# HKUST-Aerial-Robotics/D2SLAM

Hardware: AMD Instinct MI355X
Metric: frames/sec SuperPoint+NetVLAD+match, 640x480 stereo (higher is better)
Workload: dtype f32

## Files before the change

d2slam_amd/api.py:

```python
import ctypes as C
import os
from dataclasses import dataclass, field
from typing import List, Optional

import numpy as np

from .weights import SP_LAYERS

_HERE = os.path.dirname(os.path.abspath(__file__))
LIB_PATH = os.path.join(_HERE, "lib", "libd2fe_hip.so")
DEV_LIB_PATH = os.path.join(_HERE, "lib", "libd2fe_hip_dev.so")
if os.environ.get("D2FE_LIB"):
    LIB_PATH = os.path.abspath(os.environ["D2FE_LIB"])

POSTPROC_B, POSTPROC_A = 0, 1
PREC_F32, PREC_F16X2, PREC_F32_WINO, PREC_F16 = 0, 1, 2, 3
ERR_TRUNCATED = -4
KEEP_ALL_CAP = 1024
PROF_STAGES = ["conv1a", "conv1b", "conv2a", "conv2b", "conv3a", "conv3b", "conv4a", "conv4b", "convPaDa",
               "convPb", "convDb", "softmax_cand", "select", "sample", "match", "netvlad", "lk"]


class D2FEError(RuntimeError):
    def __init__(self, code, msg):
# ... 191 lines not shown
    "d2fe_lk_stereo_workspace_bytes", "d2fe_lk_track_stereo_device", "d2fe_pipe_lk_result_get",
    "d2fe_track_default_params", "d2fe_lk_carry_list_bytes", "d2fe_lk_carry_list_offset", "d2fe_lk_carry_step_device", "d2fe_pipe_track_result_get",
    "d2fe_pipe_set_track_params", "d2fe_pipe_camera_default", "d2fe_pipe_create_camera", "d2fe_pipe_submit_depth", "d2fe_pipe_depth_result_get", "d2fe_depth_at_device", "d2fe_lk_carry_quad_step_device", "d2fe_lk_carry_neighbour_device", "d2fe_quad_track_enable", "d2fe_quad_track_result_get",
    "d2fe_detect_fast_by_region", "d2fe_good_features_to_track", "d2fe_pipe_default_config", "d2fe_pipe_create", "d2fe_pipe_destroy",
    "d2fe_pipe_lanes", "d2fe_pipe_stream_placement", "d2fe_pipe_classify_stream", "d2fe_pipe_submit", "d2fe_pipe_wait", "d2fe_pipe_profile_enable", "d2fe_pipe_profile_read",
    "d2fe_pipe_device_view", "d2fe_pipe_device_release", "d2fe_pipe_lane_stream", "d2fe_pipe_geometry", "d2fe_pipe_handle",
    "d2fe_quad_pipe_default_config", "d2fe_quad_pipe_create", "d2fe_quad_pipe_destroy", "d2fe_quad_pipe_submit", "d2fe_quad_pipe_wait",
    "d2fe_quad_pipe_lanes", "d2fe_quad_pipe_geometry", "d2fe_quad_undistort_device",
    "d2fe_quad_device_view", "d2fe_quad_device_release", "d2fe_quad_lane_stream", "d2fe_quad_handle",
    "d2fe_quad_exchange_default_config", "d2fe_quad_exchange_create", "d2fe_quad_exchange_destroy", "d2fe_quad_exchange_enqueue", "d2fe_quad_exchange_collect",
    "d2fe_quad_exchange_jobs", "d2fe_quad_exchange_pairs", "d2fe_quad_exchange_block_bytes", "d2fe_quad_exchange_stream", "d2fe_quad_exchange_gathered", "d2fe_quad_exchange_job_layout",
    "d2fe_exchange_default_config", "d2fe_exchange_create", "d2fe_exchange_destroy", "d2fe_exchange_enqueue", "d2fe_exchange_collect", "d2fe_exchange_pairs",
    "d2fe_exchange_block_bytes", "d2fe_exchange_stream", "d2fe_exchange_gathered",
    "d2fe_window_default_config", "d2fe_window_create", "d2fe_window_create_quad", "d2fe_window_destroy", "d2fe_window_stream", "d2fe_window_push",
    "d2fe_window_push_host", "d2fe_window_retain", "d2fe_window_retain_plan", "d2fe_window_size", "d2fe_window_tags", "d2fe_window_track_device", "d2fe_window_collect",
    "d2fe_loop_default_config", "d2fe_loop_create", "d2fe_loop_create_quad", "d2fe_loop_destroy", "d2fe_loop_enqueue", "d2fe_loop_collect", "d2fe_loop_ntotal",
    "d2fe_loop_keyframes", "d2fe_loop_stream", "d2fe_loop_query_device", "d2fe_loop_add_host", "d2fe_rccl_load", "d2fe_rccl_path", "d2fe_rccl_unique_id", "d2fe_rccl_comm_init_rank", "d2fe_rccl_comm_destroy"]
DEBUG_EXPORTS = [
    "d2fe_debug_graph_count", "d2fe_debug_read", "d2fe_debug_netvlad_layer", "d2fe_debug_netvlad_stamps", "d2fe_debug_pack_wino",
    "d2fe_debug_pack_netvlad", "d2fe_debug_netvlad_tile", "d2fe_debug_conv3x3_wino", "d2fe_debug_match_stamps",
    "d2fe_debug_netvlad_plan", "d2fe_debug_regime_counts", "d2fe_debug_regime_reset",
    "d2fe_debug_softmax_cand", "d2fe_debug_select_b", "d2fe_debug_sample_b", "d2fe_debug_sample_b_pca", "d2fe_debug_nms2_a"]
REGIMES = ["wino_nt1_one", "wino_nt1_static", "wino_nt1_claimed", "wino_nt2_one", "wino_nt2_static", "wino_nt2_claimed_ring", "wino_nt2_claimed_fused1b",
           "match_nw4", "match_nw2", "nv_gmerge", "nv_front_tpw", "wino_last_grid", "wino_last_total"]


def _preload_hip_runtime():
    import importlib.util
    import sys
    if "torch" in sys.modules:
        return
    try:
        spec = importlib.util.find_spec("torch")
    except (ImportError, ValueError):
        spec = None
    if spec is not None and spec.origin:
        cand = os.path.join(os.path.dirname(spec.origin), "lib", "libamdhip64.so")
        if os.path.exists(cand):
            try:
                C.CDLL(cand, mode=C.RTLD_GLOBAL)
            except OSError:
                pass


def load_library(dev=False):
    global _lib, _dev_lib
    if dev:
# ... 1694 lines not shown
```

d2slam_amd/csrc/context.h:

```cpp
#pragma once
#include <hip/hip_runtime.h>

#include <atomic>

#include <array>
#include <deque>
#include <map>
#include <memory>
#include <mutex>
#include <string>
#include <vector>

#include "../../include/d2fe.h"
#include "kernels.h"
#include "sp_plan.h"

namespace d2fe {
int ctx_fail(int code, const std::string& msg);
}

#define HIP_TRY(expr)                                                                                       \
  do {                                                                                                      \
    hipError_t e_ = (expr);                                                                                 \
    if (e_ != hipSuccess)                                                                                   \
// ... 78 lines not shown
inline bool nv_is_tail(NvKind k) { return k == NvKind::Tail || k == NvKind::TailBlock; }

struct NvLayer {
  int kind, cin, cout, cout_pad, stride, act, res; int oh = 0, ow = 0;
  int gmax = 1;
  bool materialised = false;
  float* w = nullptr; float* b = nullptr;
};
struct NvStep {
  NvKind kind = NvKind::Pw; int l0 = 0, l1 = 0;
  int halves = 1;
  bool one_slab_out = false;
  float* w0 = nullptr; float* we = nullptr; float* wp = nullptr; float* bp = nullptr;
  float* wp2 = nullptr; float* bp2 = nullptr;
};
struct NvKnobs {
  static int positive(int v, int dflt) { return v > 0 ? v : dflt; }
  bool legacy = d2fe_dev_env("D2FE_NV_LEGACY", 0) != 0;
  bool pair = d2fe_dev_env("D2FE_NV_PAIR", 1) != 0, xblock = d2fe_dev_env("D2FE_NV_XBLOCK", 1) != 0;
  int blocks_target = positive(d2fe_dev_env("D2FE_NV_BLOCKS", 0), 512);
  int tail_blocks = positive(d2fe_dev_env("D2FE_NV_TAIL_BLOCKS", 0), 30);
  int slabsum = d2fe_dev_env("D2FE_NV_SLABSUM", 3);
  bool group_rule = d2fe_dev_env("D2FE_NV_GROUP_RULE", 1) != 0;
  bool merge = d2fe_dev_env("D2FE_NV_MERGE", 1) != 0;
  int front_tpw = d2fe_dev_env("D2FE_NV_FRONT_TPW", 0), nbuf = d2fe_dev_env("D2FE_NV_NBUF", 0);
  int stamp_step = d2fe_dev_env("D2FE_NV_STAMP_STEP", -1);
};
struct NvNet {
  std::vector<NvLayer> layers;
  std::vector<NvStep> plan;
  int feat = 0, proj = 0, k = 0, feat_gmax = 1;
  float *pre_w = nullptr, *pre_b = nullptr, *aw = nullptr, *aw_pack = nullptr, *ab = nullptr, *cen = nullptr;
  float *pca_comp = nullptr, *pca_mean = nullptr; int pca_m = 0;
  NvKnobs knobs;
  NvNet() = default; NvNet(const NvNet&) = delete; NvNet& operator=(const NvNet&) = delete; ~NvNet();
};
struct NvSlabs { int n = 1; long stride = 0; };
struct NvLast { std::vector<NvSlabs> layer; NvSlabs feat; int stamp_wgs = 0; };
struct NvRun {
  std::vector<float*> out;
  float *feat_buf = nullptr, *raw = nullptr, *part = nullptr;
  unsigned long long* stamps = nullptr;
  NvLast last;
  int alloc(const NvNet& net, int max_batch);
  void release();
  NvRun() = default; NvRun(const NvRun&) = delete; NvRun& operator=(const NvRun&) = delete; ~NvRun() { release(); }
// ... 125 lines not shown
```

d2slam_amd/csrc/kernels.h:

```cpp
#pragma once
#include <hip/hip_runtime.h>
#include <stdint.h>

#ifdef D2FE_DEVTOOLS
#include <cstdlib>
static inline int d2fe_dev_env(const char* name, int dflt) { const char* e = getenv(name); return e ? atoi(e) : dflt; }
#define D2FE_ABL(a, bits) ((a).ablate & (bits))
#define D2FE_STAMP(buf, wg, i) do { if ((buf) && threadIdx.x == 0) (buf)[(size_t)(wg) * 16 + (i)] = wall_clock64(); } while (0)
#else
static inline int d2fe_dev_env(const char*, int dflt) { return dflt; }
#define D2FE_ABL(a, bits) (0)
#define D2FE_STAMP(buf, wg, i) do {} while (0)
#endif

#ifdef D2FE_DEVTOOLS
#include "../../include/d2fe_debug.h"
namespace d2fe { void regime_note(int regime); void regime_set(int regime, long long value); }
#define D2FE_REGIME(r) ::d2fe::regime_note(r)
#define D2FE_REGIME_SET(r, v) ::d2fe::regime_set(r, v)
#else
#define D2FE_REGIME(r) do {} while (0)
#define D2FE_REGIME_SET(r, v) do {} while (0)
#endif

// ... 92 lines not shown

struct NvBlockArgs {
  const float* in;
  int in_slabs; long in_slab_stride;
  const uint8_t* img; int img_stride; long img_istride; int H0, W0;
  int c0_stride, c0_pt, c0_pl, act0; const float* w0;
  float* out; long out_slab_stride;
  const float* res; int res_slabs; long res_slab_stride;
  int H, W, Cin, Chid, Cout, stride, Ho, Wo, pt, pl;
  int co0, Cv;
  long P;
  int th, tw;
  unsigned inv_iw, inv_tw;
  int cpg;
  int gmerge;
  const float* we;
  const float* wp;
  const float* bp;
  int act_e, act_d, act_p;
  int ncu;
  int tpw;
  int nbuf;
  unsigned long long* stamps;
};
bool nv_block_supported(int cin, int chid, int cout, int stride, bool expand, int mode);
int nv_block_ntiles(int cout);
hipError_t launch_nv_block(const NvBlockArgs& a, bool expand, int mode, int n, int groups, hipStream_t s);
void pack_nv_expand(const float* w , const float* b, int chid, int cin, float* dst);
size_t pack_nv_expand_floats(int chid, int cin);
void pack_nv_dwproj(const float* wd , const float* bd, const float* wp , int cout, int chid, int nt, float* dst);
size_t pack_nv_dwproj_floats(int chid, int nt);
void pack_nv_proj_t(const float* wp, int cout, int chid, int nt, float* dst);
void pack_nv_dwproj_x(const float* wd, const float* bd, const float* wp, int cout, int chid, int nt, float* dst);
void pack_nv_expand_tail(const float* w, const float* b, int chid, int cin, float* dst);
bool nv_tail_supported(int cin, int cout);
hipError_t launch_nv_tail(const NvBlockArgs& a, int groups, hipStream_t s);
bool nv_xblock_supported(int cin, int chid, int cout, int stride);
void nv_xblock_tile(int Ho, int Wo, int stride, int* th, int* tw);
size_t pack_nv_expand_perm_floats(int chid, int cin);
void pack_nv_expand_perm(const float* w, const float* b, int chid, int cin, float* dst);
hipError_t launch_nv_xblock(const NvBlockArgs& a, int n, int groups, hipStream_t s);
bool nv_pblock_supported(int cin, int chid, int cout, int stride);
void nv_pblock_tile(int Ho, int Wo, int* th, int* tw, int c0_stride = 0);
size_t pack_nv_expand_pair_floats(int chid, int cin);
void pack_nv_expand_pair(const float* w, const float* b, int chid, int cin, float* dst);
size_t pack_nv_dwproj_pair_floats(int chid, int nt);
void pack_nv_dwproj_pair(const float* wd, const float* bd, const float* wp, int cout, int chid, int nt, float* dst, int co0 = 0);
int nv_pblock_ntiles(int cout);
int nv_pblock_halves(int cout);
int nv_pblock_half_cout(int cout, int half);
bool nv_pblock_single_input(int cin);
hipError_t launch_nv_pblock(const NvBlockArgs& a, int n, int groups, hipStream_t s);
bool nv_fpair_supported(int c0_cout, int c0_stride, int dw_stride, int cout);
hipError_t launch_nv_fpair(const NvBlockArgs& a, int n, hipStream_t s);
long nv_pblock_slots(int cin, int cout, int ncu, int nbuf);
hipError_t launch_nv_slab_sum(float* t, int slabs, long slab_stride, long count, hipStream_t s, int tree = 1);
bool nv_pblock_can_merge(int cin, int cv);
void pack_nv_conv0(const float* w , const float* b, int cout, float* dst );

hipError_t launch_gen_map(const double* cam9, const double* q4, int mode, int width, int height, double f, float* mapx,
                          float* mapy, hipStream_t s);
hipError_t launch_prep_gray(const uint8_t* src, int ch, int sw, int sh, int sstride, long src_istride, int n, int dw, int dh,
                            uint8_t* dst, hipStream_t s);
hipError_t launch_undistort(const uint8_t* src, int sh, int sw, int sstride, long src_istride, const float* mapx,
                            const float* mapy, const float* gain, int dh, int dw, int n, uint8_t* dst, hipStream_t s);
hipError_t launch_db_search(const float* db, int ntotal, int dim, const float* q, int nq, int k, float* sims_scratch,
                            int32_t* labels, float* out_sims, hipStream_t s);
hipError_t launch_quant_int8(const float* x, int n, int double_max, int8_t* out, hipStream_t s);
hipError_t launch_dequant_int8(const int8_t* q, int n, int landmark_num, float* out, hipStream_t s);

hipError_t launch_pack_blocks(const float* desc, const float* kps, const float* scores, const int32_t* n_kp, const float* gdesc,
                              int row0, int row_step, int nframes, int cap, int D, int G, int blk_words, float* blocks, hipStream_t s);
hipError_t launch_gate_pairs(const float* q, long q_stride, const float* db, long db_stride, int dim, const int32_t* pair_q,
                             const int32_t* pair_db, int npairs, double thres, int32_t* cnt_inout, int32_t* pass, float* sims,
                             int32_t* n_pass, hipStream_t s);
hipError_t launch_pack_blocks_int8(const float* desc, const float* kps, const int32_t* n_kp, const float* gdesc, int row0, int row_step,
                                   int nframes, int cap, int D, int G, int blk_bytes, int8_t* blocks, hipStream_t s);
hipError_t launch_unpack_blocks_int8(const int8_t* blocks, int nblocks, int cap, int D, int G, int blk_bytes, int blk_words, int renorm, float* out,
                                     hipStream_t s);
// ... 33 lines not shown
```

d2slam_amd/csrc/netvlad_host.hip:

```cpp
#include <hip/hip_runtime.h>

#include <algorithm>
#include <cstring>

#include "context.h"
#ifdef D2FE_DEVTOOLS
#include "../../include/d2fe_debug.h"
#endif

using namespace d2fe;

namespace d2fe {
NvNet::~NvNet() {
  for (auto& l : layers) for (float* p : {l.w, l.b}) if (p) hipFree(p);
  for (auto& st : plan) for (float* p : {st.w0, st.we, st.wp, st.bp, st.wp2, st.bp2}) if (p) hipFree(p);
  for (float* p : {pre_w, pre_b, aw, aw_pack, ab, cen, pca_comp, pca_mean}) if (p) hipFree(p);
}

int NvRun::alloc(const NvNet& net, int B) {
  release();
  out.assign(net.layers.size(), nullptr);
  last = {std::vector<NvSlabs>(net.layers.size()), NvSlabs(), 0};
  for (size_t li = 0; li < net.layers.size(); ++li)
    if (net.layers[li].materialised) HIP_TRY(hipMalloc(&out[li], sizeof(float) * (size_t)net.layers[li].gmax * B * net.layers[li].oh * net.layers[li].ow * net.layers[li].cout));
// ... 237 lines not shown
    else if (k == NvKind::XBlock) nv_xblock_tile(a.Ho, a.Wo, a.stride, &a.th, &a.tw);
    const long tiles1 = (long)((a.Wo + a.tw - 1) / a.tw) * ((a.Ho + a.th - 1) / a.th);
    const long tiles = tiles1 * n;
    nv_groups(tiles1, a.Chid / 16, pj.gmax, &groups, &cpg, kn.blocks_target,
              (k == NvKind::PBlock || k == NvKind::FPair) ? nv_pblock_slots(a.Cin, a.Cout, h->ncu_dev, 1) * 85 / 100 : 0, st.one_slab_out, kn.group_rule);
    a.cpg = cpg; a.out = run.out[st.l1]; a.out_slab_stride = (long)n * a.Ho * a.Wo * a.Cout;
    int tree = 1, wgroups = groups;
    const int half0 = nv_pblock_half_cout(a.Cout, 0);
    if (k == NvKind::PBlock && groups >= 6 && nv_pblock_can_merge(a.Cin, half0) && (st.halves == 1 || nv_pblock_can_merge(a.Cin, a.Cout - half0))) {
      tree = 3;
      const long slots = nv_pblock_slots(a.Cin, a.Cout, h->ncu_dev, 1);
      if (kn.merge && tiles * groups > slots && tiles * ((groups + tree - 1) / tree) * 2 >= (h->ncu_dev > 0 ? h->ncu_dev : 256)) { a.gmerge = tree; wgroups = (groups + tree - 1) / tree; }
    }
    NvSlabs& slabs = run.last.layer[st.l1];
    slabs = {wgroups, a.out_slab_stride};
    a.ncu = h->ncu; a.tpw = kn.front_tpw; a.nbuf = kn.nbuf;
    if ((int)si == kn.stamp_step && run.stamps && (tiles * wgroups <= 32768)) {
      HIP_TRY(hipMemsetAsync(run.stamps, 0, sizeof(unsigned long long) * 32 * 32768, s));
      a.stamps = run.stamps; run.last.stamp_wgs = (int)(tiles * wgroups);
    }
    switch (k) {
      case NvKind::FPair: HIP_TRY(launch_nv_fpair(a, n, s)); break;
      case NvKind::PBlock: {
        NvBlockArgs h1 = a;
        if (st.halves == 2) { a.co0 = 0; a.Cv = half0; h1.co0 = half0; h1.Cv = a.Cout - half0; h1.wp = st.wp2; h1.bp = st.bp2; h1.stamps = nullptr; }
        HIP_TRY(launch_nv_pblock(a, n, groups, s));
        if (st.halves == 2) HIP_TRY(launch_nv_pblock(h1, n, groups, s));
        break;
      }
      case NvKind::XBlock: HIP_TRY(launch_nv_xblock(a, n, groups, s)); break;
      case NvKind::Front: HIP_TRY(launch_nv_block(a, false, 1, n, groups, s)); break;
      case NvKind::Expand: HIP_TRY(launch_nv_block(a, true, 0, n, groups, s)); break;
      default: HIP_TRY(launch_nv_block(a, false, 0, n, groups, s)); break;
    }
    if (tree > 1 || (kn.slabsum > 0 && groups >= kn.slabsum) || (st.one_slab_out && groups > 1)) {
      HIP_TRY(launch_nv_slab_sum(a.out, wgroups, slabs.stride, slabs.stride, s, a.gmerge > 1 ? 1 : tree));
      slabs.n = 1;
    }
    ch = a.Ho; cw = a.Wo;
  }
  const int np = ch * cw;
  if (!feat_done) {
    const int pp = (net.proj + 31) / 32 * 32;
    HIP_TRY(launch_nv_pw(run.out.back(), (long)n * np, net.feat, net.proj, pp, 0, net.pre_w, net.pre_b, nullptr, run.feat_buf, s));
    run.last.feat = NvSlabs();
  }
// ... 185 lines not shown
```

d2slam_amd/csrc/netvlad_pair.hip:

```cpp
#include <algorithm>

#include "kernels.h"

namespace d2fe {

typedef float f32x4 __attribute__((ext_vector_type(4)));
typedef float f32x2 __attribute__((ext_vector_type(2)));

namespace {
__device__ __forceinline__ float nvp_lo(int act) { return act >= 1 ? 0.f : -__builtin_inff(); }
__device__ __forceinline__ float nvp_hi(int act) { return act == 2 ? 6.f : __builtin_inff(); }
__device__ __forceinline__ float nvp_clamp(float v, float lo, float hi) { return __builtin_amdgcn_fmed3f(v, lo, hi); }
}

constexpr int NVP_EROW = 256, NVP_EBUF = 16 * NVP_EROW, NVP_PATCH = 192;
constexpr int NVP_U8_PITCH = 40, NVP_U8_ROWS = 24, NVP_U8_DUMMY = 2 * NVP_U8_PITCH + 8;
__host__ __device__ constexpr int nvp_we_rec(int nk) { return (nk * 64 + 16 + 255) / 256 * 256; }
__host__ __device__ constexpr int nvp_rem_width(int nt) { return nt % 4 == 3 ? 4 : nt % 4; }
__host__ __device__ constexpr int nvp_ks_floats(int nt) { return 64 * (4 * (nt / 4) + nvp_rem_width(nt)); }
__host__ __device__ constexpr int nvp_wd_rec(int nt) { return (256 + 4 * nvp_ks_floats(nt) + 255) / 256 * 256; }
__host__ __device__ constexpr int nvp_row(int c) { return c * NVP_EROW + 4 * (c & 7) + 32 * (c >> 3); }

__host__ __device__ constexpr int nvp_min_waves(int nt, int nk, bool merge = false) { return (merge && nt * 8 + nk * 3 > 72) ? 2 : nt == 1 ? (nk <= 4 ? 5 : nk <= 8 ? 4 : 3) : nt == 2 ? (nk == 6 ? 4 : nk <= 8 ? 3 : 2) : (nt <= 5 && nk <= 12) ? 3 : 2; }
__host__ __device__ constexpr bool nvp_multi_in(int nk) { return nk < 18; }
template <int NT>
__device__ __forceinline__ void nvp_project(const float* wks, int lane, float d0, float d1, f32x4 (&acc)[2][NT]) {
  constexpr int NG4 = NT / 4, REM = NT % 4;
#pragma unroll
  for (int hf = 0; hf < NG4; ++hf) {
    const f32x4 v = *reinterpret_cast<const f32x4*>(wks + (hf * 64 + lane) * 4);
#pragma unroll
    for (int e = 0; e < 4; ++e) {
      acc[0][hf * 4 + e] = __builtin_amdgcn_mfma_f32_16x16x4f32(d0, v[e], acc[0][hf * 4 + e], 0, 0, 0);
      acc[1][hf * 4 + e] = __builtin_amdgcn_mfma_f32_16x16x4f32(d1, v[e], acc[1][hf * 4 + e], 0, 0, 0);
    }
  }
  if constexpr (REM != 0) {
    float wv[REM];
    const float* wr = wks + NG4 * 256;
    if constexpr (REM == 3) { const f32x4 v = *reinterpret_cast<const f32x4*>(wr + lane * 4); wv[0] = v[0]; wv[1] = v[1]; wv[2] = v[2]; }
    else if constexpr (REM == 2) { const f32x2 v = *reinterpret_cast<const f32x2*>(wr + lane * 2); wv[0] = v[0]; wv[1] = v[1]; }
    else wv[0] = wr[lane];
#pragma unroll
    for (int e = 0; e < REM; ++e) {
      acc[0][NG4 * 4 + e] = __builtin_amdgcn_mfma_f32_16x16x4f32(d0, wv[e], acc[0][NG4 * 4 + e], 0, 0, 0);
      acc[1][NG4 * 4 + e] = __builtin_amdgcn_mfma_f32_16x16x4f32(d1, wv[e], acc[1][NG4 * 4 + e], 0, 0, 0);
    }
  }
}

template <int NT, int NK, int NBUF, int MERGE = 0>
__global__ __launch_bounds__(256) __attribute__((amdgpu_waves_per_eu(nvp_min_waves(NT, NK, MERGE == 1)))) void nv_pblock_kernel(NvBlockArgs a) {
  extern __shared__ __attribute__((aligned(16))) float lds[];
  constexpr int WE_N = nvp_we_rec(NK), WD_N = nvp_wd_rec(NT), WER = WE_N / 256, WDR = WD_N / 256;
  constexpr int NK4 = NK / 4, NK2 = (NK % 4) / 2, KSF = nvp_ks_floats(NT);
  static_assert(NK % 2 == 0, "Cin must be a multiple of 8");
  const int tid = threadIdx.x, lane = tid & 63, wave = tid >> 6;
  const int lq = lane >> 4, lp = lane & 15;
  float* E = lds;
  float* WE = E + NBUF * NVP_EBUF;
  float* WD = WE + 2 * WE_N;
  const int Cin = a.Cin, Cout = a.Cout, Cv = a.Cv, th = a.th, tw = a.tw, pw = tw >> 1;
  const int iw = tw + 2, npx = (th + 2) * iw;
  const int tiles_x = (a.Wo + tw - 1) / tw;
  const int n = blockIdx.y;
  const int ty = (int)blockIdx.x / tiles_x;
  const int oy0 = ty * th, ox0 = ((int)blockIdx.x - ty * tiles_x) * tw;
  const int iy0 = oy0 - a.pt, ix0 = ox0 - a.pl;
  const int nchunk = a.Chid >> 4;
  const int wspan = MERGE ? a.gmerge * a.cpg : a.cpg;
  const int ch0 = blockIdx.z * wspan, ch1 = min(nchunk, ch0 + wspan);
  const bool lead = blockIdx.z == 0;
  unsigned long long* stamp = a.stamps ? a.stamps + (((size_t)blockIdx.z * gridDim.y + blockIdx.y) * gridDim.x + blockIdx.x) * 32 : nullptr;
  int stamp_i = 0;
  auto STAMP = [&]() { if (stamp && tid == 0 && stamp_i < 32) stamp[stamp_i] = wall_clock64(); ++stamp_i; };
  STAMP();

  const float* rp = (a.res && lead) ? a.res + (size_t)n * a.Ho * a.Wo * Cout : nullptr;
  constexpr bool RES_EARLY = !MERGE && NT <= 4 && NK < 12;
  float resv[2][4][RES_EARLY ? NT : 1];
  int obase[4];
  bool ok2[4];
#pragma unroll
  for (int r = 0; r < 4; ++r) {
    const int P = wave * 16 + lq * 4 + r;
    const int oy = (int)(((unsigned)P * a.inv_tw) >> 20), px = P - oy * pw;
    const int gy = oy0 + oy, gx = ox0 + 2 * px;
    const bool okp = P < th * pw && gy < a.Ho && gx < a.Wo;
    obase[r] = okp ? (gy * a.Wo + gx) * Cout + a.co0 + lp : -1;
    ok2[r] = okp && gx + 1 < a.Wo;
  }
  float bvv[NT];
#pragma unroll
  for (int t = 0; t < NT; ++t) bvv[t] = a.bp[t * 16 + lp];
  f32x4 tot[2][MERGE == 1 ? NT : 1];
  if constexpr (MERGE == 1) {
#pragma unroll
    for (int m2 = 0; m2 < 2; ++m2)
#pragma unroll
      for (int t = 0; t < NT; ++t)
#pragma unroll
        for (int r = 0; r < 4; ++r) {
// ... 194 lines not shown
    STAMP();
    const float* wd = WD + wb_i * WD_N;
    const float* r0 = Eb + rd0;
    const float* r1 = r0 + iw;
    const float* r2 = r1 + iw;
#pragma unroll
    for (int ks = 0; ks < 4; ++ks) {
      const f32x4 wa = *reinterpret_cast<const f32x4*>(wd + (lq * 4 + ks) * 12);
      const f32x4 wb = *reinterpret_cast<const f32x4*>(wd + (lq * 4 + ks) * 12 + 4);
      const f32x4 wc = *reinterpret_cast<const f32x4*>(wd + (lq * 4 + ks) * 12 + 8);
      const float tap[9] = {wa[0], wa[1], wa[2], wa[3], wb[0], wb[1], wb[2], wb[3], wc[0]};
      f32x2 d = {wc[1], wc[1]};
      const float* rr[3] = {r0, r1, r2};
#pragma unroll
      for (int ky = 0; ky < 3; ++ky) {
        const f32x2 A = *reinterpret_cast<const f32x2*>(rr[ky] + ks * 260);
        const f32x2 B = *reinterpret_cast<const f32x2*>(rr[ky] + ks * 260 + 2);
        d = __builtin_elementwise_fma(A, f32x2{tap[ky * 3], tap[ky * 3]}, d);
        d = __builtin_elementwise_fma(f32x2{A[1], B[0]}, f32x2{tap[ky * 3 + 1], tap[ky * 3 + 1]}, d);
        d = __builtin_elementwise_fma(B, f32x2{tap[ky * 3 + 2], tap[ky * 3 + 2]}, d);
      }
      d[0] = nvp_clamp(d[0], lo_d, hi_d); d[1] = nvp_clamp(d[1], lo_d, hi_d);
      nvp_project<NT>(wd + 256 + ks * KSF, lane, d[0], d[1], acc);
    }
    if constexpr (MERGE == 1) {
      if (--gleft == 0 || ch + 1 == ch1) {
#pragma unroll
        for (int t = 0; t < NT; ++t) {
          const float bv = (gfirst && lead) ? bvv[t] : 0.f;
#pragma unroll
          for (int m2 = 0; m2 < 2; ++m2) {
#pragma unroll
            for (int r = 0; r < 4; ++r) tot[m2][t][r] = (acc[m2][t][r] + bv) + tot[m2][t][r];
            acc[m2][t] = f32x4{0.f, 0.f, 0.f, 0.f};
          }
        }
        gleft = a.cpg; gfirst = false;
      }
    }
    STAMP();
    if (ch + 1 < ch1) store_wd(wb_i ^ 1);
    if (ch + 2 < ch1) fetch_wd(ch + 2);
    STAMP();
  }

  float* op = a.out + (size_t)blockIdx.z * a.out_slab_stride + (size_t)n * a.Ho * a.Wo * Cout;
  const float lo_p = nvp_lo(a.act_p), hi_p = nvp_hi(a.act_p);
#pragma unroll
  for (int t = 0; t < NT; ++t) {
    if (t * 16 + lp >= Cv) continue;
    const float bv = lead ? bvv[t] : 0.f;
#pragma unroll
    for (int m2 = 0; m2 < 2; ++m2)
#pragma unroll
      for (int r = 0; r < 4; ++r) {
        if (obase[r] < 0 || (m2 == 1 && !ok2[r])) continue;
        const int o = obase[r] + m2 * Cout + t * 16;
        if constexpr (MERGE == 1) { op[o] = nvp_clamp(tot[m2][t][r], lo_p, hi_p); continue; }
        float v = acc[m2][t][r] + bv;
        if constexpr (RES_EARLY) { if (rp) v += resv[m2][r][t]; }
        else if (rp) { float rs = rp[o]; for (int sl = 1; sl < a.res_slabs; ++sl) rs += rp[(size_t)sl * a.res_slab_stride + o]; v += rs; }
        op[o] = nvp_clamp(v, lo_p, hi_p);
      }
  }
  STAMP();
}

template <int NT, int NCH>
__global__ __launch_bounds__(256) __attribute__((amdgpu_waves_per_eu(NT == 1 ? (NCH == 1 ? 7 : 5) : NT == 2 ? (NCH == 1 ? 5 : 4) : NT <= 4 ? 4 : 2))) void nv_fpair_kernel(NvBlockArgs a) {
  extern __shared__ __attribute__((aligned(16))) float lds[];
  constexpr int WD_N = nvp_wd_rec(NT), WDR = NCH * WD_N / 256, KSF = nvp_ks_floats(NT);
  const int tid = threadIdx.x, lane = tid & 63, wave = tid >> 6;
  const int lq = lane >> 4, lp = lane & 15;
  float* E = lds;
  float* WD = E + NVP_EBUF;
  float* W0 = WD + NCH * WD_N;
  uint8_t* U8 = reinterpret_cast<uint8_t*>(W0 + NCH * 192);
  const int Cout = a.Cout, th = a.th, tw = a.tw, pw = tw >> 1;
  const int iw = tw + 2, npx = (th + 2) * iw;
  const int tiles_x = (a.Wo + tw - 1) / tw, ntiles = tiles_x * ((a.Ho + th - 1) / th);
  const int n = blockIdx.y;
  const int cs = a.c0_stride;
  const int UH = (th + 1) * cs + 3, UW = (iw - 1) * cs + 3;
  const int tpw = a.tpw > 0 ? a.tpw : 1;
  const int t_begin = (int)blockIdx.x * tpw, t_end = min(ntiles, t_begin + tpw);
  unsigned long long* stamp = a.stamps ? a.stamps + ((size_t)blockIdx.y * gridDim.x + blockIdx.x) * 32 : nullptr;
// ... 208 lines not shown
  const int rec = nvp_wd_rec(nt), ksf = nvp_ks_floats(nt), ng4 = nt / 4, rem = nt % 4, remw = nvp_rem_width(nt);
  for (int ch = 0; ch < (chid + 15) / 16; ++ch) {
    float* d = dst + (size_t)ch * rec;
    for (int i = 0; i < rec; ++i) d[i] = 0.f;
    for (int lq = 0; lq < 4; ++lq)
      for (int ks = 0; ks < 4; ++ks) {
        const int c = ch * 16 + ks + 4 * (lq >> 1) + 8 * (lq & 1);
        if (c >= chid) continue;
        for (int t = 0; t < 9; ++t) d[(lq * 4 + ks) * 12 + t] = wd[(size_t)c * 9 + t];
        d[(lq * 4 + ks) * 12 + 9] = bd[c];
      }
    for (int ks = 0; ks < 4; ++ks)
      for (int l = 0; l < 64; ++l) {
        const int lq = l >> 4, k = ch * 16 + ks + 4 * (lq >> 1) + 8 * (lq & 1);
        auto W = [&](int t) { const int co = t * 16 + (l & 15); return (co < cout && k < chid) ? wp[(size_t)(co0 + co) * chid + k] : 0.f; };
        float* dk = d + 256 + ks * ksf;
        for (int hf = 0; hf < ng4; ++hf)
          for (int e = 0; e < 4; ++e) dk[(hf * 64 + l) * 4 + e] = W(hf * 4 + e);
        for (int e = 0; e < rem; ++e) dk[ng4 * 256 + l * remw + e] = W(ng4 * 4 + e);
      }
  }
}

template <int NT, int NK, int NBUF, int MERGE = 0>
static hipError_t launch_pblock_b(const NvBlockArgs& a, int n, int groups, hipStream_t s) {
  const size_t lds = sizeof(float) * (NBUF * (size_t)NVP_EBUF + 2 * nvp_we_rec(NK) + 2 * nvp_wd_rec(NT));
  auto k = nv_pblock_kernel<NT, NK, NBUF, MERGE>;
  hipError_t e = hipFuncSetAttribute(reinterpret_cast<const void*>(k), hipFuncAttributeMaxDynamicSharedMemorySize, (int)lds);
  if (e != hipSuccess) return e;
  const long tiles = (long)((a.Wo + a.tw - 1) / a.tw) * ((a.Ho + a.th - 1) / a.th);
  hipLaunchKernelGGL(k, dim3((unsigned)tiles, n, groups), dim3(256), lds, s, a);
  return hipGetLastError();
}
static size_t nvp_lds_bytes(int nt, int nk, int nbuf) { return sizeof(float) * ((size_t)nbuf * NVP_EBUF + 2 * nvp_we_rec(nk) + 2 * nvp_wd_rec(nt)); }
long nv_pblock_slots(int cin, int cout, int ncu, int nbuf) {
  const int nt = nv_pblock_ntiles(nv_pblock_half_cout(cout, 0)), nk = cin / 4;
  const long per_cu = std::min<long>(nvp_min_waves(nt, nk), (long)((160 * 1024) / nvp_lds_bytes(nt, nk, nbuf)));
  return (long)(ncu > 0 ? ncu : 256) * per_cu;
}
template <int NT, int NK, int MERGE = 0>
static hipError_t launch_pblock_t(const NvBlockArgs& a, int n, int groups, hipStream_t s) {
  const int force = a.nbuf;
  const long wgs = (long)((a.Wo + a.tw - 1) / a.tw) * ((a.Ho + a.th - 1) / a.th) * n * groups;
  const bool one = force ? force == 1 : wgs * 100 > nv_pblock_slots(a.Cin, a.Cout, a.ncu, 2) * 85;
  return one ? launch_pblock_b<NT, NK, 1, MERGE>(a, n, groups, s) : launch_pblock_b<NT, NK, 2, MERGE>(a, n, groups, s);
}
#define NVP_SHAPES(X) \
  X(2, 1) X(2, 2) X(2, 4) X(2, 8) X(4, 1) X(4, 2) X(4, 4) X(4, 8) X(6, 1) X(6, 2) X(6, 3) X(6, 4) X(6, 8) X(8, 1) X(8, 2) X(8, 4) X(8, 8) \
  X(12, 3) X(12, 4) X(12, 5) X(14, 1) X(14, 2) X(14, 4) X(14, 7) X(14, 8) X(18, 5) X(18, 8) X(30, 7) X(30, 8)
#define NVP_MERGE_SHAPES(X) X(12, 3, 1) X(18, 5, 1)
bool nv_pblock_can_merge(int cin, int cv) {
  const int nk = cin / 4, nt = nv_pblock_ntiles(cv);
#define X(K, T, M) if (nk == K && nt == T) return true;
  NVP_MERGE_SHAPES(X)
#undef X
  return false;
}
static bool nvp_shape_exists(int nk, int nt) {
#define X(K, T) if (nk == K && nt == T) return true;
  NVP_SHAPES(X)
#undef X
  return false;
}
bool nv_fpair_supported(int c0_cout, int c0_stride, int dw_stride, int cout) {
  const int nt = nv_pblock_ntiles(cout);
  return (c0_cout == 16 || c0_cout == 24 || c0_cout == 32) && (c0_stride == 1 || c0_stride == 2) && dw_stride == 1 && (nt == 1 || nt == 2 || nt == 4 || nt == 8);
}
template <int NT, int NCH>
static hipError_t launch_fpair_t(const NvBlockArgs& a, int n, hipStream_t s) {
  const size_t lds = sizeof(float) * ((size_t)NVP_EBUF + NCH * (nvp_wd_rec(NT) + 192)) + NVP_U8_ROWS * NVP_U8_PITCH + NVP_U8_DUMMY;
  auto k = nv_fpair_kernel<NT, NCH>;
  hipError_t e = hipFuncSetAttribute(reinterpret_cast<const void*>(k), hipFuncAttributeMaxDynamicSharedMemorySize, (int)lds);
  if (e != hipSuccess) return e;
// ... 14 lines not shown
  if ((a.th + 1) * a.c0_stride + 3 > NVP_U8_ROWS || (a.tw + 1) * a.c0_stride + 3 > NVP_U8_PITCH) return hipErrorInvalidValue;
  const int iw = a.tw + 2, pw = a.tw / 2;
  a.inv_iw = ((1u << 20) + iw - 1) / iw; a.inv_tw = ((1u << 20) + pw - 1) / pw;
  if ((long)a.H0 * a.img_stride >= (1l << 31) || (long)a.Ho * a.Wo * a.Cout >= (1l << 31)) return hipErrorInvalidValue;
  const bool two = a.Chid > 16;
  switch (nv_pblock_ntiles(a.Cout)) {
    case 1: return two ? launch_fpair_t<1, 2>(a, n, s) : launch_fpair_t<1, 1>(a, n, s);
    case 2: return two ? launch_fpair_t<2, 2>(a, n, s) : launch_fpair_t<2, 1>(a, n, s);
    case 4: return two ? launch_fpair_t<4, 2>(a, n, s) : launch_fpair_t<4, 1>(a, n, s);
    case 8: return two ? launch_fpair_t<8, 2>(a, n, s) : launch_fpair_t<8, 1>(a, n, s);
  }
  return hipErrorInvalidValue;
}
hipError_t launch_nv_pblock(const NvBlockArgs& a_in, int n, int groups, hipStream_t s) {
  NvBlockArgs a = a_in;
  if (a.stride != 1 || a.tw < 2 || (a.tw & 1) || a.th < 1 || a.th * a.tw > 128 || (a.th + 2) * (a.tw + 2) > NVP_PATCH) return hipErrorInvalidValue;
  const int iw = a.tw + 2, pw = a.tw / 2;
  a.inv_iw = ((1u << 20) + iw - 1) / iw; a.inv_tw = ((1u << 20) + pw - 1) / pw;
  if ((long)a.H * a.W * a.Cin >= (1l << 31) || (long)a.Ho * a.Wo * a.Cout >= (1l << 31)) return hipErrorInvalidValue;
  if (a.Cv <= 0) { a.Cv = a.Cout; a.co0 = 0; }
  if (a.co0 < 0 || a.co0 + a.Cv > a.Cout || a.Cv > 128) return hipErrorInvalidValue;
  const int nk = a.Cin / 4, nt = nv_pblock_ntiles(a.Cv);
  if (a.in_slabs > 1 && !nvp_multi_in(nk)) return hipErrorInvalidValue;
  if (a.gmerge > 1) {
    const int wg = (groups + a.gmerge - 1) / a.gmerge;
    D2FE_REGIME(D2FE_REGIME_NV_GMERGE);
#define X(K, T, M) if (nk == K && nt == T) return launch_pblock_t<T, K, M>(a, n, wg, s);
    NVP_MERGE_SHAPES(X)
#undef X
    return hipErrorInvalidValue;
  }
#define X(K, T) if (nk == K && nt == T) return launch_pblock_t<T, K>(a, n, groups, s);
  NVP_SHAPES(X)
#undef X
  return hipErrorInvalidValue;
}

}
```

include/d2fe_debug.h:

```cpp
#ifndef D2FE_DEBUG_H_
#define D2FE_DEBUG_H_

#include "d2fe.h"

#ifdef __cplusplus
extern "C" {
#endif

D2FE_API long d2fe_debug_read(d2fe_handle h, const char* name, void* dst, size_t max_bytes);
D2FE_API long d2fe_debug_netvlad_layer(d2fe_handle h, int layer, int n_images, void* dst, size_t max_bytes);
D2FE_API long d2fe_debug_netvlad_stamps(d2fe_handle h, unsigned long long* dst, long max_wgs);
D2FE_API int d2fe_debug_netvlad_plan(const d2fe_nv_layer* layers, int n_layers, int proj_dim, int* out, int max_steps);
D2FE_API int d2fe_debug_netvlad_tile(int kind, int Ho, int Wo, int stride, int* th, int* tw);
D2FE_API long d2fe_debug_pack_netvlad(int kind, const float* we, const float* be, const float* wd, const float* bd, const float* wp, int cin, int chid,
                                      int cout, float* out, long max_floats);
D2FE_API long d2fe_debug_pack_wino(const float* weight , int cout, int cin, float* out, long max_floats);
D2FE_API int d2fe_debug_conv3x3_wino(d2fe_handle h, const float* in, int n, int H, int W, int cin, const float* weight,
                                     const float* bias, int cout, int pool, int relu, float* out, int iters, float* ms_per_launch);

D2FE_API int d2fe_debug_softmax_cand(d2fe_handle h, const float* logits, int lstride, int n, int Hc, int Wc, float thr, int border, int want_semi,
                                     float* semi_out, unsigned long long* cand_out, int* cand_count_out);
D2FE_API int d2fe_debug_select_b(d2fe_handle h, const unsigned long long* cand, const int* cand_count, long cand_cap, int n, int W, int H, int max_kp, int cap,
                                 int always_sort, const float* semi_or_null, float thr, int border, float* kps_xy, float* scores, int32_t* kps_idx,
                                 int32_t* n_out);
D2FE_API int d2fe_debug_sample_b(d2fe_handle h, const float* desc_raw, int dstride, int dcoff, int n, int Hc, int Wc, const float* kps_xy, const int32_t* n_kp,
                                 int cap, const int32_t* slotmap_or_null, int max_slots, float* desc_out);
D2FE_API int d2fe_debug_sample_b_pca(d2fe_handle h, const float* desc_raw, int dstride, int dcoff, int n, int Hc, int Wc, const float* kps_xy,
                                     const int32_t* n_kp, int cap, const int32_t* slotmap_or_null, int max_slots, const float* comp, const float* mean,
                                     int pca_dims, float* desc_out);
D2FE_API int d2fe_debug_nms2_a(d2fe_handle h, const float* semi, int n, int H, int W, float thr, int dist, int max_kp, int cap, float* kps_xy, float* scores,
                               int32_t* kps_idx, int32_t* n_out);

D2FE_API int d2fe_debug_graph_count(d2fe_handle h, int* rejected);

enum d2fe_regime {
  D2FE_REGIME_WINO_NT1_ONE = 0,
  D2FE_REGIME_WINO_NT1_STATIC,
  D2FE_REGIME_WINO_NT1_CLAIMED,
  D2FE_REGIME_WINO_NT2_ONE,
  D2FE_REGIME_WINO_NT2_STATIC,
  D2FE_REGIME_WINO_NT2_CLAIMED_RING,
  D2FE_REGIME_WINO_NT2_CLAIMED_FUSED1B,
  D2FE_REGIME_MATCH_NW4,
  D2FE_REGIME_MATCH_NW2,
  D2FE_REGIME_NV_GMERGE,
  D2FE_REGIME_NV_FRONT_TPW,
  D2FE_REGIME_WINO_LAST_GRID,
  D2FE_REGIME_WINO_LAST_TOTAL,
  D2FE_REGIME_COUNT
};
D2FE_API int d2fe_debug_regime_counts(long long* out, int max);
D2FE_API void d2fe_debug_regime_reset(void);

D2FE_API long d2fe_debug_match_stamps(d2fe_handle h, unsigned long long* dst, long max_wgs);

#ifdef __cplusplus
}
#endif
#endif
```

Baseline: 2325.

## Fuse both output halves of wide NetVLAD projection block into one kernel

For the two-half projection block (nk=30, nt=8, nt2=7), one kernel now computes both halves instead of launching twice. The depthwise outputs for up to three channel groups are kept in LDS and reused for a second MFMA projection pass with the second half's weights. This removes the second launch and the repeated expand/depthwise work, at the cost of extra LDS (possibly lower occupancy) and more register pressure.

```diff
diff --git a/d2slam_amd/api.py b/d2slam_amd/api.py
--- a/d2slam_amd/api.py
+++ b/d2slam_amd/api.py
@@ -237,7 +237,7 @@
     "d2fe_debug_netvlad_plan", "d2fe_debug_regime_counts", "d2fe_debug_regime_reset",
     "d2fe_debug_softmax_cand", "d2fe_debug_select_b", "d2fe_debug_sample_b", "d2fe_debug_sample_b_pca", "d2fe_debug_nms2_a"]
 REGIMES = ["wino_nt1_one", "wino_nt1_static", "wino_nt1_claimed", "wino_nt2_one", "wino_nt2_static", "wino_nt2_claimed_ring", "wino_nt2_claimed_fused1b",
-           "match_nw4", "match_nw2", "nv_gmerge", "nv_front_tpw", "wino_last_grid", "wino_last_total"]
+           "match_nw4", "match_nw2", "nv_gmerge", "nv_front_tpw", "nv_wide", "wino_last_grid", "wino_last_total"]
 
 
 def _preload_hip_runtime():
diff --git a/d2slam_amd/csrc/context.h b/d2slam_amd/csrc/context.h
--- a/d2slam_amd/csrc/context.h
+++ b/d2slam_amd/csrc/context.h
@@ -124,6 +124,7 @@
   int tail_blocks = positive(d2fe_dev_env("D2FE_NV_TAIL_BLOCKS", 0), 30);
   int slabsum = d2fe_dev_env("D2FE_NV_SLABSUM", 3);
   bool group_rule = d2fe_dev_env("D2FE_NV_GROUP_RULE", 1) != 0;
+  bool wide = d2fe_dev_env("D2FE_NV_WIDE", 1) != 0;
   bool merge = d2fe_dev_env("D2FE_NV_MERGE", 1) != 0;
   int front_tpw = d2fe_dev_env("D2FE_NV_FRONT_TPW", 0), nbuf = d2fe_dev_env("D2FE_NV_NBUF", 0);
   int stamp_step = d2fe_dev_env("D2FE_NV_STAMP_STEP", -1);
diff --git a/d2slam_amd/csrc/kernels.h b/d2slam_amd/csrc/kernels.h
--- a/d2slam_amd/csrc/kernels.h
+++ b/d2slam_amd/csrc/kernels.h
@@ -138,6 +138,7 @@
   int tpw;
   int nbuf;
   unsigned long long* stamps;
+  const float* wp2; const float* bp2; int Cv2;
 };
 bool nv_block_supported(int cin, int chid, int cout, int stride, bool expand, int mode);
 int nv_block_ntiles(int cout);
@@ -169,8 +170,9 @@
 hipError_t launch_nv_pblock(const NvBlockArgs& a, int n, int groups, hipStream_t s);
 bool nv_fpair_supported(int c0_cout, int c0_stride, int dw_stride, int cout);
 hipError_t launch_nv_fpair(const NvBlockArgs& a, int n, hipStream_t s);
-long nv_pblock_slots(int cin, int cout, int ncu, int nbuf);
+long nv_pblock_slots(int cin, int cout, int ncu, int nbuf, bool keep = false);
 hipError_t launch_nv_slab_sum(float* t, int slabs, long slab_stride, long count, hipStream_t s, int tree = 1);
+bool nv_pblock_can_keep(int cin, int cv, int cv2, int cpg);
 bool nv_pblock_can_merge(int cin, int cv);
 void pack_nv_conv0(const float* w , const float* b, int cout, float* dst );
 
diff --git a/d2slam_amd/csrc/netvlad_host.hip b/d2slam_amd/csrc/netvlad_host.hip
--- a/d2slam_amd/csrc/netvlad_host.hip
+++ b/d2slam_amd/csrc/netvlad_host.hip
@@ -283,6 +283,11 @@
     switch (k) {
       case NvKind::FPair: HIP_TRY(launch_nv_fpair(a, n, s)); break;
       case NvKind::PBlock: {
+        if (st.halves == 2 && kn.wide && a.gmerge <= 1 && nv_pblock_can_keep(a.Cin, half0, a.Cout - half0, cpg)) {
+          a.co0 = 0; a.Cv = half0; a.Cv2 = a.Cout - half0; a.wp2 = st.wp2; a.bp2 = st.bp2;
+          HIP_TRY(launch_nv_pblock(a, n, groups, s));
+          break;
+        }
         NvBlockArgs h1 = a;
         if (st.halves == 2) { a.co0 = 0; a.Cv = half0; h1.co0 = half0; h1.Cv = a.Cout - half0; h1.wp = st.wp2; h1.bp = st.bp2; h1.stamps = nullptr; }
         HIP_TRY(launch_nv_pblock(a, n, groups, s));
diff --git a/d2slam_amd/csrc/netvlad_pair.hip b/d2slam_amd/csrc/netvlad_pair.hip
--- a/d2slam_amd/csrc/netvlad_pair.hip
+++ b/d2slam_amd/csrc/netvlad_pair.hip
@@ -23,6 +23,21 @@
 
 __host__ __device__ constexpr int nvp_min_waves(int nt, int nk, bool merge = false) { return (merge && nt * 8 + nk * 3 > 72) ? 2 : nt == 1 ? (nk <= 4 ? 5 : nk <= 8 ? 4 : 3) : nt == 2 ? (nk == 6 ? 4 : nk <= 8 ? 3 : 2) : (nt <= 5 && nk <= 12) ? 3 : 2; }
 __host__ __device__ constexpr bool nvp_multi_in(int nk) { return nk < 18; }
+constexpr int NVP_KEEP = 3;
+template <int NT>
+__device__ __forceinline__ void nvp_bfrag(const float* wks, int lane, float (&wv)[NT]) {
+  constexpr int NG4 = NT / 4, REM = NT % 4;
+#pragma unroll
+  for (int hf = 0; hf < NG4; ++hf) {
+    const f32x4 v = *reinterpret_cast<const f32x4*>(wks + (hf * 64 + lane) * 4);
+#pragma unroll
+    for (int e = 0; e < 4; ++e) wv[hf * 4 + e] = v[e];
+  }
+  const float* wr = wks + NG4 * 256;
+  if constexpr (REM == 3) { const f32x4 v = *reinterpret_cast<const f32x4*>(wr + lane * 4); wv[NG4 * 4] = v[0]; wv[NG4 * 4 + 1] = v[1]; wv[NG4 * 4 + 2] = v[2]; }
+  else if constexpr (REM == 2) { const f32x2 v = *reinterpret_cast<const f32x2*>(wr + lane * 2); wv[NG4 * 4] = v[0]; wv[NG4 * 4 + 1] = v[1]; }
+  else if constexpr (REM == 1) wv[NG4 * 4] = wr[lane];
+}
 template <int NT>
 __device__ __forceinline__ void nvp_project(const float* wks, int lane, float d0, float d1, f32x4 (&acc)[2][NT]) {
   constexpr int NG4 = NT / 4, REM = NT % 4;
@@ -49,8 +64,9 @@
   }
 }
 
-template <int NT, int NK, int NBUF, int MERGE = 0>
+template <int NT, int NK, int NBUF, int MERGE = 0, int NT2 = 0>
 __global__ __launch_bounds__(256) __attribute__((amdgpu_waves_per_eu(nvp_min_waves(NT, NK, MERGE == 1)))) void nv_pblock_kernel(NvBlockArgs a) {
+  static_assert(NT2 == 0 || (MERGE == 0 && NT > 4), "no second project phase with a running total or an early residual");
   extern __shared__ __attribute__((aligned(16))) float lds[];
   constexpr int WE_N = nvp_we_rec(NK), WD_N = nvp_wd_rec(NT), WER = WE_N / 256, WDR = WD_N / 256;
   constexpr int NK4 = NK / 4, NK2 = (NK % 4) / 2, KSF = nvp_ks_floats(NT);
@@ -60,6 +76,7 @@
   float* E = lds;
   float* WE = E + NBUF * NVP_EBUF;
   float* WD = WE + 2 * WE_N;
+  float* DK = WD + 2 * WD_N;
   const int Cin = a.Cin, Cout = a.Cout, Cv = a.Cv, th = a.th, tw = a.tw, pw = tw >> 1;
   const int iw = tw + 2, npx = (th + 2) * iw;
   const int tiles_x = (a.Wo + tw - 1) / tw;
@@ -77,7 +94,7 @@
   STAMP();
 
   const float* rp = (a.res && lead) ? a.res + (size_t)n * a.Ho * a.Wo * Cout : nullptr;
-  constexpr bool RES_EARLY = !MERGE && NT <= 4 && NK < 12;
+  constexpr bool RES_EARLY = !MERGE && NT2 == 0 && NT <= 4 && NK < 12;
   float resv[2][4][RES_EARLY ? NT : 1];
   int obase[4];
   bool ok2[4];
@@ -318,6 +335,7 @@
       }
       d[0] = nvp_clamp(d[0], lo_d, hi_d); d[1] = nvp_clamp(d[1], lo_d, hi_d);
       nvp_project<NT>(wd + 256 + ks * KSF, lane, d[0], d[1], acc);
+      if constexpr (NT2 > 0) *reinterpret_cast<f32x2*>(DK + (((ch - ch0) * 4 + ks) * 256 + tid) * 2) = d;
     }
     if constexpr (MERGE == 1) {
       if (--gleft == 0 || ch + 1 == ch1) {
@@ -342,22 +360,71 @@
 
   float* op = a.out + (size_t)blockIdx.z * a.out_slab_stride + (size_t)n * a.Ho * a.Wo * Cout;
   const float lo_p = nvp_lo(a.act_p), hi_p = nvp_hi(a.act_p);
-#pragma unroll
-  for (int t = 0; t < NT; ++t) {
-    if (t * 16 + lp >= Cv) continue;
-    const float bv = lead ? bvv[t] : 0.f;
-#pragma unroll
-    for (int m2 = 0; m2 < 2; ++m2)
-#pragma unroll
-      for (int r = 0; r < 4; ++r) {
-        if (obase[r] < 0 || (m2 == 1 && !ok2[r])) continue;
-        const int o = obase[r] + m2 * Cout + t * 16;
-        if constexpr (MERGE == 1) { op[o] = nvp_clamp(tot[m2][t][r], lo_p, hi_p); continue; }
-        float v = acc[m2][t][r] + bv;
-        if constexpr (RES_EARLY) { if (rp) v += resv[m2][r][t]; }
-        else if (rp) { float rs = rp[o]; for (int sl = 1; sl < a.res_slabs; ++sl) rs += rp[(size_t)sl * a.res_slab_stride + o]; v += rs; }
-        op[o] = nvp_clamp(v, lo_p, hi_p);
-      }
+  if constexpr (NT2 == 0) {
+#pragma unroll
+    for (int t = 0; t < NT; ++t) {
+      if (t * 16 + lp >= Cv) continue;
+      const float bv = lead ? bvv[t] : 0.f;
+#pragma unroll
+      for (int m2 = 0; m2 < 2; ++m2)
+#pragma unroll
+        for (int r = 0; r < 4; ++r) {
+          if (obase[r] < 0 || (m2 == 1 && !ok2[r])) continue;
+          const int o = obase[r] + m2 * Cout + t * 16;
+          if constexpr (MERGE == 1) { op[o] = nvp_clamp(tot[m2][t][r], lo_p, hi_p); continue; }
+          float v = acc[m2][t][r] + bv;
+          if constexpr (RES_EARLY) { if (rp) v += resv[m2][r][t]; }
+          else if (rp) { float rs = rp[o]; for (int sl = 1; sl < a.res_slabs; ++sl) rs += rp[(size_t)sl * a.res_slab_stride + o]; v += rs; }
+          op[o] = nvp_clamp(v, lo_p, hi_p);
+        }
+    }
+  } else {
+    auto store_half = [&](const auto& ac, const float* bias, int c_off, int cv) {
+      constexpr int N = sizeof(ac[0]) / sizeof(f32x4);
+#pragma unroll
+      for (int t = 0; t < N; ++t) {
+        if (t * 16 + lp >= cv) continue;
+        const float bv = lead ? bias[t] : 0.f;
+#pragma unroll
+        for (int m2 = 0; m2 < 2; ++m2)
+#pragma unroll
+          for (int r = 0; r < 4; ++r) {
+            if (obase[r] < 0 || (m2 == 1 && !ok2[r])) continue;
+            const int o = obase[r] + m2 * Cout + c_off + t * 16;
+            float v = ac[m2][t][r] + bv;
+            if (rp) { float rs = rp[o]; for (int sl = 1; sl < a.res_slabs; ++sl) rs += rp[(size_t)sl * a.res_slab_stride + o]; v += rs; }
+            op[o] = nvp_clamp(v, lo_p, hi_p);
+          }
+      }
+    };
+    constexpr int WD2_N = nvp_wd_rec(NT2), KSF2 = nvp_ks_floats(NT2);
+    float w2[NVP_KEEP][4][NT2], bv2[NT2];
+#pragma unroll
+    for (int j = 0; j < NVP_KEEP; ++j)
+      if (ch0 + j < ch1)
+#pragma unroll
+        for (int ks = 0; ks < 4; ++ks) nvp_bfrag<NT2>(a.wp2 + (size_t)(ch0 + j) * WD2_N + 256 + ks * KSF2, lane, w2[j][ks]);
+#pragma unroll
+    for (int t = 0; t < NT2; ++t) bv2[t] = a.bp2[t * 16 + lp];
+    store_half(acc, bvv, 0, Cv);
+    f32x4 acc2[2][NT2];
+#pragma unroll
+    for (int m = 0; m < 2; ++m)
+#pragma unroll
+      for (int t = 0; t < NT2; ++t) acc2[m][t] = f32x4{0.f, 0.f, 0.f, 0.f};
+#pragma unroll
+    for (int j = 0; j < NVP_KEEP; ++j)
+      if (ch0 + j < ch1)
+#pragma unroll
+        for (int ks = 0; ks < 4; ++ks) {
+          const f32x2 d = *reinterpret_cast<const f32x2*>(DK + ((j * 4 + ks) * 256 + tid) * 2);
+#pragma unroll
+          for (int t = 0; t < NT2; ++t) {
+            acc2[0][t] = __builtin_amdgcn_mfma_f32_16x16x4f32(d[0], w2[j][ks][t], acc2[0][t], 0, 0, 0);
+            acc2[1][t] = __builtin_amdgcn_mfma_f32_16x16x4f32(d[1], w2[j][ks][t], acc2[1][t], 0, 0, 0);
+          }
+        }
+    store_half(acc2, bv2, Cv, a.Cv2);
   }
   STAMP();
 }
@@ -612,33 +679,42 @@
   }
 }
 
-template <int NT, int NK, int NBUF, int MERGE = 0>
+static size_t nvp_lds_bytes(int nt, int nk, int nbuf, bool keep = false) { return sizeof(float) * ((size_t)nbuf * NVP_EBUF + 2 * nvp_we_rec(nk) + 2 * nvp_wd_rec(nt) + (keep ? NVP_KEEP * 2048 : 0)); }
+template <int NT, int NK, int NBUF, int MERGE = 0, int NT2 = 0>
 static hipError_t launch_pblock_b(const NvBlockArgs& a, int n, int groups, hipStream_t s) {
-  const size_t lds = sizeof(float) * (NBUF * (size_t)NVP_EBUF + 2 * nvp_we_rec(NK) + 2 * nvp_wd_rec(NT));
-  auto k = nv_pblock_kernel<NT, NK, NBUF, MERGE>;
+  const size_t lds = nvp_lds_bytes(NT, NK, NBUF, NT2 > 0);
+  auto k = nv_pblock_kernel<NT, NK, NBUF, MERGE, NT2>;
   hipError_t e = hipFuncSetAttribute(reinterpret_cast<const void*>(k), hipFuncAttributeMaxDynamicSharedMemorySize, (int)lds);
   if (e != hipSuccess) return e;
   const long tiles = (long)((a.Wo + a.tw - 1) / a.tw) * ((a.Ho + a.th - 1) / a.th);
   hipLaunchKernelGGL(k, dim3((unsigned)tiles, n, groups), dim3(256), lds, s, a);
   return hipGetLastError();
 }
-static size_t nvp_lds_bytes(int nt, int nk, int nbuf) { return sizeof(float) * ((size_t)nbuf * NVP_EBUF + 2 * nvp_we_rec(nk) + 2 * nvp_wd_rec(nt)); }
-long nv_pblock_slots(int cin, int cout, int ncu, int nbuf) {
+long nv_pblock_slots(int cin, int cout, int ncu, int nbuf, bool keep) {
   const int nt = nv_pblock_ntiles(nv_pblock_half_cout(cout, 0)), nk = cin / 4;
-  const long per_cu = std::min<long>(nvp_min_waves(nt, nk), (long)((160 * 1024) / nvp_lds_bytes(nt, nk, nbuf)));
+  const long per_cu = std::min<long>(nvp_min_waves(nt, nk), (long)((160 * 1024) / nvp_lds_bytes(nt, nk, nbuf, keep)));
   return (long)(ncu > 0 ? ncu : 256) * per_cu;
 }
-template <int NT, int NK, int MERGE = 0>
+template <int NT, int NK, int MERGE = 0, int NT2 = 0>
 static hipError_t launch_pblock_t(const NvBlockArgs& a, int n, int groups, hipStream_t s) {
   const int force = a.nbuf;
   const long wgs = (long)((a.Wo + a.tw - 1) / a.tw) * ((a.Ho + a.th - 1) / a.th) * n * groups;
-  const bool one = force ? force == 1 : wgs * 100 > nv_pblock_slots(a.Cin, a.Cout, a.ncu, 2) * 85;
-  return one ? launch_pblock_b<NT, NK, 1, MERGE>(a, n, groups, s) : launch_pblock_b<NT, NK, 2, MERGE>(a, n, groups, s);
+  const bool one = force ? force == 1 : wgs * 100 > nv_pblock_slots(a.Cin, a.Cout, a.ncu, 2, NT2 > 0) * 85;
+  return one ? launch_pblock_b<NT, NK, 1, MERGE, NT2>(a, n, groups, s) : launch_pblock_b<NT, NK, 2, MERGE, NT2>(a, n, groups, s);
 }
 #define NVP_SHAPES(X) \
   X(2, 1) X(2, 2) X(2, 4) X(2, 8) X(4, 1) X(4, 2) X(4, 4) X(4, 8) X(6, 1) X(6, 2) X(6, 3) X(6, 4) X(6, 8) X(8, 1) X(8, 2) X(8, 4) X(8, 8) \
   X(12, 3) X(12, 4) X(12, 5) X(14, 1) X(14, 2) X(14, 4) X(14, 7) X(14, 8) X(18, 5) X(18, 8) X(30, 7) X(30, 8)
 #define NVP_MERGE_SHAPES(X) X(12, 3, 1) X(18, 5, 1)
+#define NVP_KEEP_SHAPES(X) X(30, 8, 7)
+bool nv_pblock_can_keep(int cin, int cv, int cv2, int cpg) {
+  const int nk = cin / 4, nt = nv_pblock_ntiles(cv), nt2 = nv_pblock_ntiles(cv2);
+  if (cpg > NVP_KEEP || cv != nt * 16) return false;
+#define X(K, T, T2) if (nk == K && nt == T && nt2 == T2) return true;
+  NVP_KEEP_SHAPES(X)
+#undef X
+  return false;
+}
 bool nv_pblock_can_merge(int cin, int cv) {
   const int nk = cin / 4, nt = nv_pblock_ntiles(cv);
 #define X(K, T, M) if (nk == K && nt == T) return true;
@@ -699,6 +775,14 @@
   if (a.co0 < 0 || a.co0 + a.Cv > a.Cout || a.Cv > 128) return hipErrorInvalidValue;
   const int nk = a.Cin / 4, nt = nv_pblock_ntiles(a.Cv);
   if (a.in_slabs > 1 && !nvp_multi_in(nk)) return hipErrorInvalidValue;
+  if (a.Cv2 > 0) {
+    if (a.gmerge > 1 || a.co0 != 0 || a.Cv + a.Cv2 > a.Cout || !a.wp2 || !a.bp2 || !nv_pblock_can_keep(a.Cin, a.Cv, a.Cv2, a.cpg)) return hipErrorInvalidValue;
+    D2FE_REGIME(D2FE_REGIME_NV_WIDE);
+#define X(K, T, T2) if (nk == K && nt == T && nv_pblock_ntiles(a.Cv2) == T2) return launch_pblock_t<T, K, 0, T2>(a, n, groups, s);
+    NVP_KEEP_SHAPES(X)
+#undef X
+    return hipErrorInvalidValue;
+  }
   if (a.gmerge > 1) {
     const int wg = (groups + a.gmerge - 1) / a.gmerge;
     D2FE_REGIME(D2FE_REGIME_NV_GMERGE);
diff --git a/include/d2fe_debug.h b/include/d2fe_debug.h
--- a/include/d2fe_debug.h
+++ b/include/d2fe_debug.h
@@ -45,6 +45,7 @@
   D2FE_REGIME_MATCH_NW2,
   D2FE_REGIME_NV_GMERGE,
   D2FE_REGIME_NV_FRONT_TPW,
+  D2FE_REGIME_NV_WIDE,
   D2FE_REGIME_WINO_LAST_GRID,
   D2FE_REGIME_WINO_LAST_TOTAL,
   D2FE_REGIME_COUNT
```

Measured after the change: 2329, median of 6. Within noise of the previous version (+0.2%).
